# paulmillr/noble-curves

Hardware: AMD Instinct MI355X
Metric: secp256k1_scalar_mults_per_sec (higher is better)
Workload: dtype u32

## Files before the change

### noble-curves_amd/csrc/consts_gen.hpp

```cpp
#pragma once
#include <stdint.h>
namespace ncg {

struct ParamsSecpP {
  static constexpr int N = 8;
  static constexpr uint32_t P[8] = {0xfffffc2fu, 0xfffffffeu, 0xffffffffu, 0xffffffffu, 0xffffffffu, 0xffffffffu, 0xffffffffu, 0xffffffffu};
  static constexpr uint32_t INV = 0xd2253531u;
  static constexpr uint32_t R1[8] = {0x00000001u, 0x00000000u, 0x00000000u, 0x00000000u, 0x00000000u, 0x00000000u, 0x00000000u, 0x00000000u};
  static constexpr uint32_t R2[8] = {0x00000001u, 0x00000000u, 0x00000000u, 0x00000000u, 0x00000000u, 0x00000000u, 0x00000000u, 0x00000000u};
  static constexpr bool TOP_SPARE = false;
  static constexpr bool FOLD = true;
  static constexpr uint32_t FOLD_LO = 0x000003d1u;
  static constexpr uint32_t FOLD_HI = 1u;
  static constexpr int FINAL_SUBS = 1;
  static constexpr uint32_t BETA[8] = {0x719501eeu, 0xc1396c28u, 0x12f58995u, 0x9cf04975u, 0xac3434e9u, 0x6e64479eu, 0x657c0710u, 0x7ae96a2bu};
  static constexpr uint32_t B3[8] = {0x00000015u, 0x00000000u, 0x00000000u, 0x00000000u, 0x00000000u, 0x00000000u, 0x00000000u, 0x00000000u};
};

struct ParamsEdP {
  static constexpr int N = 8;
  static constexpr uint32_t P[8] = {0xffffffedu, 0xffffffffu, 0xffffffffu, 0xffffffffu, 0xffffffffu, 0xffffffffu, 0xffffffffu, 0x7fffffffu};
  static constexpr uint32_t INV = 0x286bca1bu;
  static constexpr uint32_t R1[8] = {0x00000001u, 0x00000000u, 0x00000000u, 0x00000000u, 0x00000000u, 0x00000000u, 0x00000000u, 0x00000000u};
  static constexpr uint32_t R2[8] = {0x00000001u, 0x00000000u, 0x00000000u, 0x00000000u, 0x00000000u, 0x00000000u, 0x00000000u, 0x00000000u};
  static constexpr bool TOP_SPARE = true;
  static constexpr bool FOLD = true;
  static constexpr uint32_t FOLD_LO = 0x00000026u;
  static constexpr uint32_t FOLD_HI = 0u;
  static constexpr int FINAL_SUBS = 2;
  static constexpr uint32_t D[8] = {0x135978a3u, 0x75eb4dcau, 0x4141d8abu, 0x00700a4du, 0x7779e898u, 0x8cc74079u, 0x2b6ffe73u, 0x52036ceeu};
  static constexpr uint32_t D2[8] = {0x26b2f159u, 0xebd69b94u, 0x8283b156u, 0x00e0149au, 0xeef3d130u, 0x198e80f2u, 0x56dffce7u, 0x2406d9dcu};
  static constexpr uint32_t SQRT_M1[8] = {0x4a0ea0b0u, 0xc4ee1b27u, 0xad2fe478u, 0x2f431806u, 0x3dfbd7a7u, 0x2b4d0099u, 0x4fc1df0bu, 0x2b832480u};
};

struct ParamsBlsP {
  static constexpr int N = 12;
  static constexpr uint32_t P[12] = {0xffffaaabu, 0xb9feffffu, 0xb153ffffu, 0x1eabfffeu, 0xf6b0f624u, 0x6730d2a0u, 0xf38512bfu, 0x64774b84u, 0x434bacd7u, 0x4b1ba7b6u, 0x397fe69au, 0x1a0111eau};
  static constexpr uint32_t INV = 0xfffcfffdu;
  static constexpr uint32_t R1[12] = {0x0002fffdu, 0x76090000u, 0xc40c0002u, 0xebf4000bu, 0x53c758bau, 0x5f489857u, 0x70525745u, 0x77ce5853u, 0xa256ec6du, 0x5c071a97u, 0xfa80e493u, 0x15f65ec3u};
  static constexpr uint32_t R2[12] = {0x1c341746u, 0xf4df1f34u, 0x09d104f1u, 0x0a76e6a6u, 0x4c95b6d5u, 0x8de5476cu, 0x939d83c0u, 0x67eb88a9u, 0xb519952du, 0x9a793e85u, 0x92cae3aau, 0x11988fe5u};
  static constexpr bool TOP_SPARE = true;
  static constexpr bool FOLD = false;
};

struct Fe9SecpPR {
  static constexpr uint32_t P[9] = {0x1ffffc2fu, 0x1ffffff7u, 0x1fffffffu, 0x1fffffffu, 0x1fffffffu, 0x1fffffffu, 0x1fffffffu, 0x1fffffffu, 0x00ffffffu};
  static constexpr uint32_t C0 = 31264u, C1 = 256u;
  static constexpr uint32_t PINV = 0x0ddacacfu;
  static constexpr int JMAX = 33;
  static constexpr uint32_t BIAS[8][9] = {
    {0x00000000u, 0x00000000u, 0x00000000u, 0x00000000u, 0x00000000u, 0x00000000u, 0x00000000u, 0x00000000u, 0x00000000u},
    {0x3fff820fu, 0x3ffffef6u, 0x3ffffffeu, 0x3ffffffeu, 0x3ffffffeu, 0x3ffffffeu, 0x3ffffffeu, 0x3ffffffeu, 0x20fffffeu},
    {0x5fff07efu, 0x5ffffdf5u, 0x5ffffffdu, 0x5ffffffdu, 0x5ffffffdu, 0x5ffffffdu, 0x5ffffffdu, 0x5ffffffdu, 0x40fffffdu},
    {0x7ffe8dcfu, 0x7ffffcf4u, 0x7ffffffcu, 0x7ffffffcu, 0x7ffffffcu, 0x7ffffffcu, 0x7ffffffcu, 0x7ffffffcu, 0x60fffffcu},
    {0x9ffe13afu, 0x9ffffbf3u, 0x9ffffffbu, 0x9ffffffbu, 0x9ffffffbu, 0x9ffffffbu, 0x9ffffffbu, 0x9ffffffbu, 0x80fffffbu},
    {0xbffd998fu, 0xbffffaf2u, 0xbffffffau, 0xbffffffau, 0xbffffffau, 0xbffffffau, 0xbffffffau, 0xbffffffau, 0xa0fffffau},
    {0xdffd1f6fu, 0xdffff9f1u, 0xdffffff9u, 0xdffffff9u, 0xdffffff9u, 0xdffffff9u, 0xdffffff9u, 0xdffffff9u, 0xc0fffff9u},
    {0xfffca54fu, 0xfffff8f0u, 0xfffffff8u, 0xfffffff8u, 0xfffffff8u, 0xfffffff8u, 0xfffffff8u, 0xfffffff8u, 0xe0fffff8u},
  };
  static constexpr uint32_t BETA[9] = {0x119501eeu, 0x09cb6143u, 0x1d626570u, 0x0092ea25u, 0x034e99cfu, 0x03cf561au, 0x1c41b991u, 0x056caf80u, 0x007ae96au};
};

struct Fe9EdPR {
  static constexpr uint32_t P[9] = {0x1fffffedu, 0x1fffffffu, 0x1fffffffu, 0x1fffffffu, 0x1fffffffu, 0x1fffffffu, 0x1fffffffu, 0x1fffffffu, 0x007fffffu};
  static constexpr uint32_t C0 = 1216u, C1 = 0u;
  static constexpr uint32_t PINV = 0x179435e5u;
  static constexpr int JMAX = 65;
  static constexpr uint32_t BIAS[8][9] = {
    {0x00000000u, 0x00000000u, 0x00000000u, 0x00000000u, 0x00000000u, 0x00000000u, 0x00000000u, 0x00000000u, 0x00000000u},
    {0x3ffffb2du, 0x3ffffffeu, 0x3ffffffeu, 0x3ffffffeu, 0x3ffffffeu, 0x3ffffffeu, 0x3ffffffeu, 0x3ffffffeu, 0x207ffffeu},
    {0x5ffff66du, 0x5ffffffdu, 0x5ffffffdu, 0x5ffffffdu, 0x5ffffffdu, 0x5ffffffdu, 0x5ffffffdu, 0x5ffffffdu, 0x407ffffdu},
    {0x7ffff1adu, 0x7ffffffcu, 0x7ffffffcu, 0x7ffffffcu, 0x7ffffffcu, 0x7ffffffcu, 0x7ffffffcu, 0x7ffffffcu, 0x607ffffcu},
    {0x9fffecedu, 0x9ffffffbu, 0x9ffffffbu, 0x9ffffffbu, 0x9ffffffbu, 0x9ffffffbu, 0x9ffffffbu, 0x9ffffffbu, 0x807ffffbu},
    {0xbfffe82du, 0xbffffffau, 0xbffffffau, 0xbffffffau, 0xbffffffau, 0xbffffffau, 0xbffffffau, 0xbffffffau, 0xa07ffffau},
    {0xdfffe36du, 0xdffffff9u, 0xdffffff9u, 0xdffffff9u, 0xdffffff9u, 0xdffffff9u, 0xdffffff9u, 0xdffffff9u, 0xc07ffff9u},
    {0xffffdeadu, 0xfffffff8u, 0xfffffff8u, 0xfffffff8u, 0xfffffff8u, 0xfffffff8u, 0xfffffff8u, 0xfffffff8u, 0xe07ffff8u},
  };
  static constexpr uint32_t D[9] = {0x135978a3u, 0x0f5a6e50u, 0x10762addu, 0x00149a82u, 0x1e898007u, 0x003cbbbcu, 0x19ce331du, 0x1dc56dffu, 0x0052036cu};
  static constexpr uint32_t D2[9] = {0x06b2f159u, 0x1eb4dca1u, 0x00ec55bau, 0x00293505u, 0x1d13000eu, 0x00797779u, 0x139c663au, 0x1b8adbffu, 0x002406d9u};
  static constexpr uint32_t SQRT_M1[9] = {0x0a0ea0b0u, 0x0770d93au, 0x0bf91e31u, 0x06300d5au, 0x1d7a72f4u, 0x004c9efdu, 0x1c2cad34u, 0x1009f83bu, 0x002b8324u};
  static constexpr uint32_t SQRT_AD_MINUS_ONE[9] = {0x097b2e1bu, 0x14bfb502u, 0x1e152f5fu, 0x1b1c1836u, 0x1d1fdaf9u, 0x1e6498fau, 0x02b03cf3u, 0x17e57069u, 0x00376931u};
  static constexpr uint32_t INVSQRT_A_MINUS_D[9] = {0x005d40eau, 0x0e47ed54u, 0x105cafa6u, 0x1e2c2eb4u, 0x1d8409d2u, 0x1dc8ff00u, 0x12885b09u, 0x00b9f5ffu, 0x00786c89u};
  static constexpr uint32_t ONE_MINUS_D_SQ[9] = {0x145fc176u, 0x13e04e0cu, 0x178d43f8u, 0x0342719au, 0x0dfe42c8u, 0x15eedf38u, 0x035e6652u, 0x1516567cu, 0x00029072u};
  static constexpr uint32_t D_MINUS_ONE_SQ[9] = {0x04ed4d20u, 0x0d6ad552u, 0x0786664cu, 0x1c945960u, 0x14eebd29u, 0x0997a94du, 0x09053373u, 0x0f5ecd84u, 0x005968b3u};
};

struct ParamsBls29 {
  static constexpr int N = 14;
  static constexpr int BITS = 29;
  static constexpr uint32_t P[14] = {0x1fffaaabu, 0x0ff7ffffu, 0x14ffffeeu, 0x17fffd62u, 0x0f6241eau, 0x09507b58u, 0x0afd9cc3u, 0x109e70a2u, 0x1764774bu, 0x121a5d66u, 0x12c6e9edu, 0x12ffcd34u, 0x00111ea3u, 0x0000000du};
  static constexpr uint32_t INV = 0x1ffcfffdu;
  static constexpr uint32_t R1[14] = {0x03a9fb84u, 0x0ba00690u, 0x071288f1u, 0x0f59bcc5u, 0x126cb614u, 0x0585bf36u, 0x1b85ac3du, 0x1cf856fau, 0x1891ecbdu, 0x1a7eec05u, 0x155a88f0u, 0x0741ac6du, 0x1317c30fu, 0x00000009u};
  static constexpr uint32_t R2[14] = {0x15bef7aeu, 0x1031cd0eu, 0x02dd93e8u, 0x09226323u, 0x0e6e2cd2u, 0x11684daau, 0x1170e5dbu, 0x088e25b1u, 0x1b366399u, 0x1c536f47u, 0x0d1f9cbcu, 0x0278b67fu, 0x1ea66a2bu, 0x0000000cu};
  static constexpr uint32_t PMUL[13][14] = {
    {0x1fffaaabu, 0x0ff7ffffu, 0x14ffffeeu, 0x17fffd62u, 0x0f6241eau, 0x09507b58u, 0x0afd9cc3u, 0x109e70a2u, 0x1764774bu, 0x121a5d66u, 0x12c6e9edu, 0x12ffcd34u, 0x00111ea3u, 0x0000000du},
    {0x1fff5556u, 0x1fefffffu, 0x09ffffdcu, 0x0ffffac5u, 0x1ec483d5u, 0x12a0f6b0u, 0x15fb3986u, 0x013ce144u, 0x0ec8ee97u, 0x0434bacdu, 0x058dd3dbu, 0x05ff9a69u, 0x00223d47u, 0x0000001au},
    {0x1ffeaaacu, 0x1fdfffffu, 0x13ffffb9u, 0x1ffff58au, 0x1d8907aau, 0x0541ed61u, 0x0bf6730du, 0x0279c289u, 0x1d91dd2eu, 0x0869759au, 0x0b1ba7b6u, 0x0bff34d2u, 0x00447a8eu, 0x00000034u},
    {0x1ffd5558u, 0x1fbfffffu, 0x07ffff73u, 0x1fffeb15u, 0x1b120f55u, 0x0a83dac3u, 0x17ece61au, 0x04f38512u, 0x1b23ba5cu, 0x10d2eb35u, 0x16374f6cu, 0x17fe69a4u, 0x0088f51cu, 0x00000068u},
    {0x1ffaaab0u, 0x1f7fffffu, 0x0ffffee7u, 0x1fffd62au, 0x16241eabu, 0x1507b587u, 0x0fd9cc34u, 0x09e70a25u, 0x164774b8u, 0x01a5d66bu, 0x0c6e9ed9u, 0x0ffcd349u, 0x0111ea39u, 0x000000d0u},
    {0x1ff55560u, 0x1effffffu, 0x1ffffdcfu, 0x1fffac54u, 0x0c483d57u, 0x0a0f6b0fu, 0x1fb39869u, 0x13ce144au, 0x0c8ee970u, 0x034bacd7u, 0x18dd3db2u, 0x1ff9a692u, 0x0223d472u, 0x000001a0u},
    {0x1feaaac0u, 0x1dffffffu, 0x1ffffb9fu, 0x1fff58a9u, 0x18907aafu, 0x141ed61eu, 0x1f6730d2u, 0x079c2895u, 0x191dd2e1u, 0x069759aeu, 0x11ba7b64u, 0x1ff34d25u, 0x0447a8e5u, 0x00000340u},
    {0x1fd55580u, 0x1bffffffu, 0x1ffff73fu, 0x1ffeb153u, 0x1120f55fu, 0x083dac3du, 0x1ece61a5u, 0x0f38512bu, 0x123ba5c2u, 0x0d2eb35du, 0x0374f6c8u, 0x1fe69a4bu, 0x088f51cbu, 0x00000680u},
    {0x1faaab00u, 0x17ffffffu, 0x1fffee7fu, 0x1ffd62a7u, 0x0241eabfu, 0x107b587bu, 0x1d9cc34au, 0x1e70a257u, 0x04774b84u, 0x1a5d66bbu, 0x06e9ed90u, 0x1fcd3496u, 0x111ea397u, 0x00000d00u},
    {0x1f555600u, 0x0fffffffu, 0x1fffdcffu, 0x1ffac54fu, 0x0483d57fu, 0x00f6b0f6u, 0x1b398695u, 0x1ce144afu, 0x08ee9709u, 0x14bacd76u, 0x0dd3db21u, 0x1f9a692cu, 0x023d472fu, 0x00001a01u},
    {0x1eaaac00u, 0x1fffffffu, 0x1fffb9feu, 0x1ff58a9fu, 0x0907aaffu, 0x01ed61ecu, 0x16730d2au, 0x19c2895fu, 0x11dd2e13u, 0x09759aecu, 0x1ba7b643u, 0x1f34d258u, 0x047a8e5fu, 0x00003402u},
    {0x1d555800u, 0x1fffffffu, 0x1fff73fdu, 0x1feb153fu, 0x120f55ffu, 0x03dac3d8u, 0x0ce61a54u, 0x138512bfu, 0x03ba5c27u, 0x12eb35d9u, 0x174f6c86u, 0x1e69a4b1u, 0x08f51cbfu, 0x00006804u},
    {0x1aaab000u, 0x1fffffffu, 0x1ffee7fbu, 0x1fd62a7fu, 0x041eabffu, 0x07b587b1u, 0x19cc34a8u, 0x070a257eu, 0x0774b84fu, 0x05d66bb2u, 0x0e9ed90du, 0x1cd34963u, 0x11ea397fu, 0x0000d008u},
  };
  static constexpr uint32_t FOUR[14] = {0x0ea898bau, 0x0e901a40u, 0x124a23e8u, 0x0d66f84fu, 0x0aee547cu, 0x03760629u, 0x181b776eu, 0x12a47aa6u, 0x137ec460u, 0x05c6f549u, 0x0fdc4fe8u, 0x1707174du, 0x0c3ccef5u, 0x0000000cu};
  static constexpr uint32_t G1_BETA[14] = {0x0abf79e7u, 0x194b14ebu, 0x1ceb16a6u, 0x1845cd5du, 0x0c814568u, 0x199ca109u, 0x13ee6ee1u, 0x05d123e5u, 0x0dfbdce2u, 0x010ecb54u, 0x0d9337edu, 0x1daaf4b0u, 0x146806fbu, 0x0000000cu};
  static constexpr uint32_t HALF[14] = {0x01d4fdc2u, 0x15d00348u, 0x13894478u, 0x07acde62u, 0x09365b0au, 0x12c2df9bu, 0x0dc2d61eu, 0x1e7c2b7du, 0x1c48f65eu, 0x0d3f7602u, 0x1aad4478u, 0x13a0d636u, 0x198be187u, 0x00000004u};
  static constexpr uint32_t PSI_X_C0[14] = {0x00000000u, 0x00000000u, 0x00000000u, 0x00000000u, 0x00000000u, 0x00000000u, 0x00000000u, 0x00000000u, 0x00000000u, 0x00000000u, 0x00000000u, 0x00000000u, 0x00000000u, 0x00000000u};
  static constexpr uint32_t PSI_X_C1[14] = {0x154030c4u, 0x16aceb14u, 0x1814e947u, 0x1fba3004u, 0x02e0fc81u, 0x0fb3da4fu, 0x170f2de1u, 0x0acd4cbcu, 0x09689a69u, 0x110b9212u, 0x0533b200u, 0x1554d884u, 0x0ba917a7u, 0x00000000u};
  static constexpr uint32_t PSI_Y_C0[14] = {0x099d9feeu, 0x1cfab983u, 0x07e0b07eu, 0x1f87f0f2u, 0x0bc18573u, 0x0cdbe130u, 0x010ddd19u, 0x100cbeafu, 0x09169c21u, 0x0f93673eu, 0x11de55b3u, 0x097ddc84u, 0x11fce827u, 0x0000000cu};
  static constexpr uint32_t PSI_Y_C1[14] = {0x16620abdu, 0x12fd467cu, 0x0d1f4f6fu, 0x18780c70u, 0x03a0bc76u, 0x1c749a28u, 0x09efbfa9u, 0x0091b1f3u, 0x0e4ddb2au, 0x0286f628u, 0x00e8943au, 0x0981f0b0u, 0x0e14367cu, 0x00000000u};
  static constexpr uint64_t P58[7] = {0x01feffffffffaaabull, 0x02ffffac54ffffeeull, 0x012a0f6b0f6241eaull, 0x0213ce144afd9cc3ull, 0x02434bacd764774bull, 0x025ff9a692c6e9edull, 0x00000001a0111ea3ull};
  static constexpr uint64_t INV58 = 0x01f3fffcfffcfffdull;
};

struct BlsH2c {
  static constexpr int ISO1_XNUM_N = 12;
  static constexpr uint32_t ISO1_XNUM[12][14] = {
    {0x19533850u, 0x1fde0061u, 0x1658849cu, 0x0468a403u, 0x03312074u, 0x0755dadbu, 0x0f9d5f6au, 0x0d765d96u, 0x1f3db0ebu, 0x027072a2u, 0x0cd72ecfu, 0x192a1295u, 0x0b9df03du, 0x00000000u},
    {0x08a13a19u, 0x0e61b7a9u, 0x10c7b287u, 0x19352d6cu, 0x19fcef3au, 0x1bd60694u, 0x0b00008bu, 0x14ac9157u, 0x1bfc81b7u, 0x0cf31437u, 0x1f7ef30cu, 0x174125b4u, 0x16bc996bu, 0x00000003u},
    {0x1d34d585u, 0x001816fdu, 0x0697e05du, 0x0bd01a7fu, 0x06319923u, 0x0526b67eu, 0x127cdfdeu, 0x1c4ccaedu, 0x16999bd6u, 0x1dc05cf6u, 0x0c798715u, 0x1b067cadu, 0x0e1b22d3u, 0x00000001u},
    {0x05b95fd0u, 0x1561eeaeu, 0x0708c4e2u, 0x1ca04592u, 0x0a64d8b5u, 0x161de6c8u, 0x0ed13a80u, 0x1c0b9393u, 0x1f81aea0u, 0x1f7805d0u, 0x1f7443d4u, 0x0410f2d9u, 0x12d9db9fu, 0x00000004u},
    {0x19f42c99u, 0x19554edbu, 0x01bb4832u, 0x08df9f46u, 0x1aa4ed11u, 0x0c014ee5u, 0x0503d165u, 0x024ff2c0u, 0x014d2026u, 0x038449cbu, 0x004265aeu, 0x075ca7f4u, 0x0abdbe88u, 0x0000000cu},
    {0x06e086cbu, 0x12e06cf1u, 0x1010c3f7u, 0x097dc760u, 0x009ce362u, 0x1fdead02u, 0x03b2a43cu, 0x13dc159au, 0x12f1e75fu, 0x0c59d18bu, 0x0993cd0du, 0x17aada76u, 0x0f653a62u, 0x0000000au},
    {0x05f32e93u, 0x04de80d5u, 0x0257dd44u, 0x1b3fa578u, 0x08ad968du, 0x18f7fcf4u, 0x135a2c12u, 0x1b3437dfu, 0x1bf48b7fu, 0x027e482cu, 0x10ad5b95u, 0x1f53c6ecu, 0x13593facu, 0x0000000cu},
    {0x100e8415u, 0x00260d8au, 0x0416be13u, 0x002f5de8u, 0x12f06c69u, 0x0614ac97u, 0x078c4e2cu, 0x0f0e1a44u, 0x12527cbfu, 0x1aa0dad8u, 0x1b9d18c9u, 0x03052990u, 0x06c178c5u, 0x00000008u},
    {0x020e35ffu, 0x1509aba1u, 0x011197a7u, 0x07424063u, 0x00fdf22au, 0x1cdffda5u, 0x15e86ee3u, 0x0dc72f5eu, 0x085ed13bu, 0x17a167e6u, 0x1d4f68a3u, 0x12bc0758u, 0x0da1d102u, 0x0000000bu},
    {0x16f92abfu, 0x1d97eb20u, 0x03799de9u, 0x0afdfcdbu, 0x0593e7abu, 0x1c07c98eu, 0x113c6b21u, 0x0c6c4382u, 0x15178c4bu, 0x004d295bu, 0x160c0213u, 0x0b223d3cu, 0x138a06aeu, 0x00000005u},
    {0x0d584f0eu, 0x13abb276u, 0x114fd2fdu, 0x13587172u, 0x1c078395u, 0x19d77f56u, 0x14ed4ae3u, 0x134b5001u, 0x07368705u, 0x08ccfc06u, 0x169d5582u, 0x04364b97u, 0x1e36a0acu, 0x0000000cu},
    {0x1e2dc07eu, 0x14fb1b8eu, 0x1d54c7fdu, 0x1ffe9f96u, 0x1d9e8c8eu, 0x082c550du, 0x10f80cc9u, 0x0fbb5189u, 0x1731633cu, 0x0d2b8d78u, 0x1142fdc6u, 0x0a530186u, 0x09b1edb4u, 0x00000003u}
  };
  static constexpr int ISO1_XDEN_N = 11;
  static constexpr uint32_t ISO1_XDEN[11][14] = {
    {0x16aada94u, 0x121b61fbu, 0x17d25789u, 0x00ea9a1bu, 0x01f559e5u, 0x1977be06u, 0x17199839u, 0x0b55fcacu, 0x001b9b0eu, 0x101b75ebu, 0x0b9bd0a9u, 0x1276bf47u, 0x14703656u, 0x00000002u},
    {0x109ff044u, 0x10ea0db9u, 0x1f93b8bdu, 0x1ef8d6d2u, 0x1ad8ab3cu, 0x1cd635f7u, 0x1ebd2c90u, 0x01e90c38u, 0x12519856u, 0x1002aed7u, 0x0d3b5c6fu, 0x0cb89003u, 0x0ed3e5c4u, 0x0000000au},
    {0x0f77e4d1u, 0x08f1403du, 0x1b1578a2u, 0x134e8b79u, 0x11c5fe2au, 0x1af37000u, 0x061d1654u, 0x0f79cc45u, 0x1fcafbd1u, 0x00394301u, 0x1c85638fu, 0x02143baau, 0x0fd37998u, 0x00000007u},
    {0x16688f1eu, 0x1834f256u, 0x033c4e2eu, 0x1b7c3ab5u, 0x0aef9a87u, 0x16e2b034u, 0x04ea8170u, 0x0b5ed828u, 0x109f419cu, 0x1b1ce49fu, 0x0b8d1767u, 0x1f6a5c83u, 0x08c7b891u, 0x0000000cu},
    {0x0cfbd1b4u, 0x13f5968cu, 0x04d98113u, 0x078bb5a2u, 0x0a047c3au, 0x1f58a89au, 0x14970a3fu, 0x070dc778u, 0x05a639fau, 0x1e4df2a1u, 0x15236253u, 0x006cbe19u, 0x0747e1aau, 0x00000000u},
    {0x1ba56c55u, 0x0da2285eu, 0x1bdde522u, 0x1323e0bfu, 0x14fcd4dfu, 0x160d9669u, 0x126e3cb8u, 0x1ae38ab4u, 0x043ccd6cu, 0x1c50479du, 0x03ccf828u, 0x14a8dc86u, 0x0baa345eu, 0x00000005u},
    {0x1763cc52u, 0x1af364d0u, 0x0d599836u, 0x01b13b47u, 0x19625c2cu, 0x0c93c70fu, 0x1981cf56u, 0x16ce23d0u, 0x116786d9u, 0x1b64f75fu, 0x0396c2e5u, 0x17ce2455u, 0x137ac25cu, 0x0000000cu},
    {0x135eaa4eu, 0x11a0ee2cu, 0x1c8ae208u, 0x04908755u, 0x0742ff48u, 0x1aa65057u, 0x1ccabcc6u, 0x0ca2e07cu, 0x0a7fdbf0u, 0x065f3fd1u, 0x09b8d593u, 0x11ab564eu, 0x1b009d39u, 0x0000000au},
    {0x04b0c530u, 0x0ab8267du, 0x03c5d708u, 0x0859392au, 0x05ae9638u, 0x1db0f3d5u, 0x0b1bdfc7u, 0x0c8c0cf0u, 0x192090ddu, 0x0f85b4e6u, 0x09cb08bdu, 0x0e6aeeebu, 0x05feaf09u, 0x00000005u},
    {0x0ee55d76u, 0x0fe759f8u, 0x16bac213u, 0x04ced8e4u, 0x097e4bacu, 0x19215e96u, 0x1d46ea21u, 0x145404aeu, 0x11ade63fu, 0x0c8756c9u, 0x031fc337u, 0x15c18a0eu, 0x1fcb94acu, 0x00000005u},
    {0x03a9fb84u, 0x0ba00690u, 0x071288f1u, 0x0f59bcc5u, 0x126cb614u, 0x0585bf36u, 0x1b85ac3du, 0x1cf856fau, 0x1891ecbdu, 0x1a7eec05u, 0x155a88f0u, 0x0741ac6du, 0x1317c30fu, 0x00000009u}
  };
  static constexpr int ISO1_YNUM_N = 16;
// ... 144 lines not shown
```

### noble-curves_amd/csrc/fe9.hpp

```cpp
#pragma once
#include <type_traits>

#include "fp.hpp"
#include "fe9_asm_gen.hpp"
#include "fe9m.hpp"

namespace ncg {

constexpr uint32_t FE9_MASK = (1u << 29) - 1u;

template <class PR, class = void> struct Fe9IsMont : std::false_type {};
template <class PR> struct Fe9IsMont<PR, std::void_t<decltype(PR::MONT)>> : std::integral_constant<bool, PR::MONT> {};

template <class PR>
struct Fe9Raw {
  uint32_t v[9];
};

NCG_DI void fe9_mac(uint64_t& acc, uint32_t a, uint32_t b) {
#ifdef __HIP_DEVICE_COMPILE__
  asm("v_mad_u64_u32 %0, vcc, %1, %2, %0" : "+v"(acc) : "v"(a), "v"(b) : "vcc");
#else
  acc += (uint64_t)a * b;
#endif
// ... 458 lines not shown
  int32_t bw = 0;
#pragma unroll
  for (int i = 0; i < 9; i++) {
    int32_t dd = (int32_t)t[i] - (int32_t)PR::P[i] + bw;
    s[i] = (uint32_t)dd & FE9_MASK;
    bw = dd >> 29;
  }
  const bool ge = bw == 0;
#pragma unroll
  for (int i = 0; i < 9; i++) o[i] = ge ? s[i] : t[i];
}

template <class PR, class... T>
__host__ __device__ __noinline__ bool fe9_eqz_slow(T... limbs) {
  Fe9<PR, 7> a;
  const uint32_t v[9] = {limbs...};
#pragma unroll
  for (int i = 0; i < 9; i++) a.v[i] = v[i];
  uint32_t c[9];
  fe9_canon_limbs<PR, 7>(c, a);
  uint32_t o = 0;
#pragma unroll
  for (int i = 0; i < 9; i++) o |= c[i];
  return o == 0;
}
template <class PR, int A>
NCG_DI bool f_eqz(const Fe9<PR, A>& a) {
  const uint32_t j = (a.v[0] * PR::PINV) & FE9_MASK;
  if (j >= (uint32_t)(PR::JMAX * A)) return false;
  return fe9_eqz_slow<PR>(a.v[0], a.v[1], a.v[2], a.v[3], a.v[4], a.v[5], a.v[6], a.v[7], a.v[8]);
}
template <class PR, int A, int B>
NCG_DI bool f_eq(const Fe9<PR, A>& a, const Fe9<PR, B>& b) {
  return f_eqz(a - b);
}

template <class PR>
NCG_DI Fe9<PR, 1> fe9_from_wire(const uint32_t* __restrict__ p) {
  if constexpr (Fe9IsMont<PR>::value) {
    Fe9<PR, 1> r;
    fe9m_from_wire(r.v, p);
    return r;
  }
  uint32_t w[10];
#pragma unroll
  for (int i = 0; i < 8; i++) w[i] = p[i];
  w[8] = 0;
  w[9] = 0;
  Fe9<PR, 1> r;
#pragma unroll
  for (int i = 0; i < 9; i++) {
    const int bit = 29 * i, limb = bit >> 5, sh = bit & 31;
    const uint64_t two = ((uint64_t)w[limb + 1] << 32) | w[limb];
    r.v[i] = (uint32_t)(two >> sh) & FE9_MASK;
  }
  return r;
}
template <class PR, int A>
NCG_DI void fe9_to_wire(uint32_t* __restrict__ p, const Fe9<PR, A>& a) {
  if constexpr (Fe9IsMont<PR>::value) {
    uint32_t c[9];
    fe9m_canon_plain(c, fe9_norm(a).v);
    fe9m_words_from_limbs(p, c);
    return;
  }
  uint32_t l[11];
  uint32_t c[9];
  fe9_canon_limbs<PR, A>(c, a);
#pragma unroll
  for (int i = 0; i < 9; i++) l[i] = c[i];
  l[9] = 0;
  l[10] = 0;
#pragma unroll
  for (int k = 0; k < 8; k++) {
    const int bit = 32 * k, limb = bit / 29, sh = bit % 29;
    uint64_t acc = (uint64_t)l[limb] >> sh;
    acc |= (uint64_t)l[limb + 1] << (29 - sh);
    acc |= (uint64_t)l[limb + 2] << (58 - sh);
    p[k] = (uint32_t)acc;
  }
}

template <class PR, int A>
NCG_DI Fe9<PR, 1> f_inv(const Fe9<PR, A>& a_in) {
  using F = Fe9<PR, 1>;
  const F x = fe9_norm(a_in);
  if constexpr (Fe9IsMont<PR>::value) {
    F tab[16];
    tab[0] = F::one();
    tab[1] = x;
#pragma unroll
    for (int i = 2; i < 16; i++) tab[i] = tab[i - 1] * x;
    F t = tab[PR::PM2_NIB[63]];
#pragma unroll
    for (int i = 62; i >= 0; i--) {
      t = fe9_sqr_n(t, 4);
      const int d = PR::PM2_NIB[i];
      if (d) t = t * tab[d];
    }
    return t;
  } else if constexpr (PR::C1 != 0) {
    F x2 = f_sqr(x) * x;
    F x3 = f_sqr(x2) * x;
    F x6 = fe9_sqr_n(x3, 3) * x3;
    F x9 = fe9_sqr_n(x6, 3) * x3;
    F x11 = fe9_sqr_n(x9, 2) * x2;
    F x22 = fe9_sqr_n(x11, 11) * x11;
    F x44 = fe9_sqr_n(x22, 22) * x22;
    F x88 = fe9_sqr_n(x44, 44) * x44;
    F x176 = fe9_sqr_n(x88, 88) * x88;
    F x220 = fe9_sqr_n(x176, 44) * x44;
    F x223 = fe9_sqr_n(x220, 3) * x3;
    F t = fe9_sqr_n(x223, 23) * x22;
    t = fe9_sqr_n(t, 5) * x;
    t = fe9_sqr_n(t, 3) * x2;
    t = fe9_sqr_n(t, 2) * x;
    return t;
  } else {
    F z2 = f_sqr(x);
    F z9 = fe9_sqr_n(z2, 2) * x;
    F z11 = z9 * z2;
    F z2_5_0 = f_sqr(z11) * z9;
    F z2_10_0 = fe9_sqr_n(z2_5_0, 5) * z2_5_0;
    F z2_20_0 = fe9_sqr_n(z2_10_0, 10) * z2_10_0;
    F z2_40_0 = fe9_sqr_n(z2_20_0, 20) * z2_20_0;
    F z2_50_0 = fe9_sqr_n(z2_40_0, 10) * z2_10_0;
    F z2_100_0 = fe9_sqr_n(z2_50_0, 50) * z2_50_0;
    F z2_200_0 = fe9_sqr_n(z2_100_0, 100) * z2_100_0;
    F z2_250_0 = fe9_sqr_n(z2_200_0, 50) * z2_50_0;
    return fe9_sqr_n(z2_250_0, 5) * z11;
  }
}

using FeSecp = Fe9<Fe9SecpPR, 2>;
using FeEd = Fe9<Fe9EdPR, 2>;
using FeBn254 = Fe9<Bn254PR, 2>;

}
```

### noble-curves_amd/csrc/hosttest.hip

```cpp
#include <vector>

#include "../../include/ncg.h"
#include "mulvar.hpp"
#include "ed25519.hip"
#include "decode.hip"
#include "ntt.hip"
#include "poly.hip"
#include "h2c.hip"
#include "endo.hpp"
#include "ecdsa.hip"
#include "msm_shard.hpp"
#include "msm_endo.hip"
#include "msm_schedule.hpp"
#include "fe9m_check.hpp"
#include "group_check.hpp"
#include "x25519.hip"
#include "ristretto.hip"

using namespace ncg;

template <class C, int W>
static void ht_mul_var_t(const uint32_t* pts, const uint32_t* scalars, uint32_t* out, uint8_t* out_inf, int n) {
  constexpr int FW = MulVarCfg<C, W>::FW, WW = MulVarCfg<C, W>::WW;
  std::vector<uint32_t> tab(MulVarCfg<C, W>::TS * 2 * FW);
// ... 185 lines not shown
  Fe9<PR, C> z;
  Fe9<PR, D> w;
  for (int i = 0; i < 9; i++) {
    x.v[i] = a[i];
    y.v[i] = b[i];
    z.v[i] = c[i];
    w.v[i] = d[i];
  }
  Fe9<PR, 1> o;
  if constexpr (A * B + C * D <= 7) {
    if (op == 0) o = f_mul_mul(x, y, z, w);
  }
  if constexpr (C <= 2 && A * B + C * C <= 7) {
    if (op == 1) o = f_mul_sqr(x, y, z);
  }
  if constexpr (A * B <= 7) {
    if (op == 2) o = f_mul_add(x, y, z);
  }
  if constexpr (A <= 2) {
    if (op == 3) o = f_sqr_add(x, z);
  }
  if constexpr (A == 1) {
    if (op == 4) {
      const Fe9<PR, 2> h = f_half(x);
      for (int i = 0; i < 9; i++) r[i] = h.v[i];
      return;
    }
  }
  for (int i = 0; i < 9; i++) r[i] = o.v[i];
}
template <class PR>
static int ht_fe9_fused_t(int op, int variant, const uint32_t* a, const uint32_t* b, const uint32_t* c, const uint32_t* d, uint32_t* r) {
  switch (variant) {
    case 1111: ht_fe9_fused_ab<PR, 1, 1, 1, 1>(op, a, b, c, d, r); return 0;
    case 1322: ht_fe9_fused_ab<PR, 1, 3, 2, 2>(op, a, b, c, d, r); return 0;
    case 3211: ht_fe9_fused_ab<PR, 3, 2, 1, 1>(op, a, b, c, d, r); return 0;
    case 2311: ht_fe9_fused_ab<PR, 2, 3, 1, 1>(op, a, b, c, d, r); return 0;
    case 1123: ht_fe9_fused_ab<PR, 1, 1, 2, 3>(op, a, b, c, d, r); return 0;
    case 3121: ht_fe9_fused_ab<PR, 3, 1, 2, 1>(op, a, b, c, d, r); return 0;
    case 1327: ht_fe9_fused_ab<PR, 1, 3, 2, 7>(op, a, b, c, d, r); return 0;
    case 7171: ht_fe9_fused_ab<PR, 7, 1, 7, 1>(op, a, b, c, d, r); return 0;
    case 1771: ht_fe9_fused_ab<PR, 1, 7, 7, 1>(op, a, b, c, d, r); return 0;
    case 2171: ht_fe9_fused_ab<PR, 2, 1, 7, 1>(op, a, b, c, d, r); return 0;
    default: return -1;
  }
}

template <class F>
static int fr29_op_host(int op, const uint32_t* a, const uint32_t* b, uint32_t* r) {
  Fr29 x, y, z;
  for (int i = 0; i < 9; i++) {
    x.v[i] = a[i];
    y.v[i] = b ? b[i] : 0;
    z.v[i] = 0;
  }
  fr29_overflows() = 0;
  switch (op) {
    case 0: z = fr29_mont<F>(x, y); break;
    case 1: z = fr29_add(x, y); break;
    case 2: z = fr29_sub<F>(x, y); break;
    case 3: z = fr29_weak(x); break;
    case 4: z = fr29_reduce256<F>(x); break;
    case 5: z = fr29_cond_sub<F>(x); break;
    case 8: z = fr29_fold255<F>(x); break;
    case 6: {
      uint32_t w[8];
      for (int i = 0; i < 8; i++) w[i] = a[i];
      z = fr29_from_words(w);
      break;
    }
    case 7: {
      uint32_t w[8];
      fr29_to_words(w, x);
      for (int i = 0; i < 8; i++) z.v[i] = w[i];
      z.v[8] = 0;
      break;
    }
    default: return -1;
  }
  for (int i = 0; i < 9; i++) r[i] = z.v[i];
  return fr29_overflows();
}

extern "C" {

int ht_fe9_op(int field, int op, int variant, const uint32_t* a, const uint32_t* b, uint32_t* r) {
  if (field == 0) return ht_fe9_t<Fe9SecpPR>(op, variant, a, b, r);
  if (field == 1) return ht_fe9_t<Fe9EdPR>(op, variant, a, b, r);
  return -1;
}

int ht_mul_var(int curve, const uint32_t* pts, const uint32_t* scalars, uint32_t* out, uint8_t* out_inf, int n) {
  switch (curve) {
    case CURVE_SECP256K1: ht_mul_var_t<CurveSecp, 4>(pts, scalars, out, out_inf, n); return 0;
    case CURVE_BLS12_381_G1: ht_mul_var_t<CurveG1, 3>(pts, scalars, out, out_inf, n); return 0;
    case 12: ht_mul_var_t<CurveG1E, 4>(pts, scalars, out, out_inf, n); return 0;
    case 14: ht_mul_var_t<CurveSecpI, 4>(pts, scalars, out, out_inf, n); return 0;
    case CURVE_BLS12_381_G2: ht_mul_var_t<CurveG2, 3>(pts, scalars, out, out_inf, n); return 0;
    case CURVE_BN254_G1: ht_mul_var_t<CurveBn254, 4>(pts, scalars, out, out_inf, n); return 0;
  }
  return -1;
}

int ht_field_op(int field, int op, const uint32_t* a, const uint32_t* b, uint32_t* r) {
  switch (field) {
    case 0: ht_field_t<ParamsSecpP>(op, a, b, r); return 0;
    case 1: ht_field_t<ParamsEdP>(op, a, b, r); return 0;
    case 2: ht_field_t<ParamsBlsP>(op, a, b, r); return 0;
  }
  return -1;
}

int ht_fe9_fused(int field, int op, int variant, const uint32_t* a, const uint32_t* b, const uint32_t* c, const uint32_t* d,
                 uint32_t* r) {
  if (field == 0) return ht_fe9_fused_t<Fe9SecpPR>(op, variant, a, b, c, d, r);
  if (field == 1) return ht_fe9_fused_t<Fe9EdPR>(op, variant, a, b, c, d, r);
  return -1;
}

int ht_jac_neg(int op, const uint32_t* p, const uint32_t* qx, const uint32_t* qy, uint32_t* out) {
  Jac<FeSecp> P;
  Fe9<Fe9SecpPR, 2> x;
  Fe9<Fe9SecpPR, 3> y;
  for (int i = 0; i < 9; i++) {
    P.X.v[i] = p[i];
    P.Y.v[i] = p[9 + i];
    P.Z.v[i] = p[18 + i];
    x.v[i] = qx[i];
    y.v[i] = qy[i];
  }
  Jac<FeSecp> R;
  if (op == 0) R = jac_dbl_neg(P);
  else if (op == 1) R = jac_madd_neg(P, x, y);
  else return -1;
  for (int i = 0; i < 9; i++) {
    out[i] = R.X.v[i];
    out[9 + i] = R.Y.v[i];
    out[18 + i] = R.Z.v[i];
  }
  return 0;
}

int ht_glv_split_odd(const uint32_t* k, uint32_t* out) {
  uint32_t kk[8];
  for (int i = 0; i < 8; i++) kk[i] = k[i];
  GlvSplit s = secp_glv_split(kk);
  secp_glv_make_odd(s);
  for (int i = 0; i < 5; i++) {
    out[i] = s.k1[i];
    out[5 + i] = s.k2[i];
  }
  out[10] = s.k1neg;
  out[11] = s.k2neg;
  return 0;
}

int ht_glv_split_k1_odd(const uint32_t* k, uint32_t* out) {
  uint32_t kk[8];
  for (int i = 0; i < 8; i++) kk[i] = k[i];
  GlvSplit s = secp_glv_split(kk);
  secp_glv_make_k1_odd(s);
  for (int i = 0; i < 5; i++) {
    out[i] = s.k1[i];
    out[5 + i] = s.k2[i];
  }
  out[10] = s.k1neg;
  out[11] = s.k2neg;
  return 0;
}

int ht_glv_split(const uint32_t* k, uint32_t* out) {
  uint32_t kk[8];
// ... 374 lines not shown
```

Measured before the change: 134.7 million.

## Replace Fermat field inversion with batched divsteps (safegcd) inversion for fe9 fields

Field inversion for non-Montgomery fe9 fields (secp256k1, ed25519) now uses a Bernstein-Yang divsteps algorithm on signed 30-bit limbs. It batches 30 divsteps per iteration with 2x2 transition matrices and exits early once the whole wavefront has g==0, falling back to Fermat inversion if the iteration cap is reached. The aim is to avoid the roughly 256 squarings plus multiplies of exponentiation. The cost is wave-uniform iteration counts and more branchy code. Host test hooks for comparing the two inversions are also added.

After: 136.8 million (median of 6 runs). +1.6%, better.

```diff
diff --git a/noble-curves_amd/csrc/consts_gen.hpp b/noble-curves_amd/csrc/consts_gen.hpp
--- a/noble-curves_amd/csrc/consts_gen.hpp
+++ b/noble-curves_amd/csrc/consts_gen.hpp
@@ -48,6 +48,8 @@
   static constexpr uint32_t C0 = 31264u, C1 = 256u;
   static constexpr uint32_t PINV = 0x0ddacacfu;
   static constexpr int JMAX = 33;
+  static constexpr int32_t P30[9] = {-977, -4, 0, 0, 0, 0, 0, 0, 65536};
+  static constexpr uint32_t PINV30 = 0x2ddacacfu;
   static constexpr uint32_t BIAS[8][9] = {
     {0x00000000u, 0x00000000u, 0x00000000u, 0x00000000u, 0x00000000u, 0x00000000u, 0x00000000u, 0x00000000u, 0x00000000u},
     {0x3fff820fu, 0x3ffffef6u, 0x3ffffffeu, 0x3ffffffeu, 0x3ffffffeu, 0x3ffffffeu, 0x3ffffffeu, 0x3ffffffeu, 0x20fffffeu},
@@ -66,6 +68,8 @@
   static constexpr uint32_t C0 = 1216u, C1 = 0u;
   static constexpr uint32_t PINV = 0x179435e5u;
   static constexpr int JMAX = 65;
+  static constexpr int32_t P30[9] = {-19, 0, 0, 0, 0, 0, 0, 0, 32768};
+  static constexpr uint32_t PINV30 = 0x179435e5u;
   static constexpr uint32_t BIAS[8][9] = {
     {0x00000000u, 0x00000000u, 0x00000000u, 0x00000000u, 0x00000000u, 0x00000000u, 0x00000000u, 0x00000000u, 0x00000000u},
     {0x3ffffb2du, 0x3ffffffeu, 0x3ffffffeu, 0x3ffffffeu, 0x3ffffffeu, 0x3ffffffeu, 0x3ffffffeu, 0x3ffffffeu, 0x207ffffeu},
diff --git a/noble-curves_amd/csrc/fe9.hpp b/noble-curves_amd/csrc/fe9.hpp
--- a/noble-curves_amd/csrc/fe9.hpp
+++ b/noble-curves_amd/csrc/fe9.hpp
@@ -564,7 +564,7 @@
 }
 
 template <class PR, int A>
-NCG_DI Fe9<PR, 1> f_inv(const Fe9<PR, A>& a_in) {
+NCG_DI Fe9<PR, 1> f_inv_fermat(const Fe9<PR, A>& a_in) {
   using F = Fe9<PR, 1>;
   const F x = fe9_norm(a_in);
   if constexpr (Fe9IsMont<PR>::value) {
@@ -614,6 +614,16 @@
   }
 }
 
+}
+#include "fe9_inv.hpp"
+namespace ncg {
+
+template <class PR, int A>
+NCG_DI Fe9<PR, 1> f_inv(const Fe9<PR, A>& a_in) {
+  if constexpr (Fe9IsMont<PR>::value) return f_inv_fermat(a_in);
+  else return fe9_inv_divsteps(a_in);
+}
+
 using FeSecp = Fe9<Fe9SecpPR, 2>;
 using FeEd = Fe9<Fe9EdPR, 2>;
 using FeBn254 = Fe9<Bn254PR, 2>;
diff --git a/noble-curves_amd/csrc/fe9_inv.hpp b/noble-curves_amd/csrc/fe9_inv.hpp
--- /dev/null
+++ b/noble-curves_amd/csrc/fe9_inv.hpp
@@ -0,0 +1,192 @@
+#pragma once
+
+namespace ncg {
+
+constexpr uint32_t FE9_M30 = (1u << 30) - 1u;
+constexpr int FE9_DS_CAP = 20;
+
+NCG_DI bool fe9_wave_any(bool c) {
+#ifdef __HIP_DEVICE_COMPILE__
+  return __builtin_amdgcn_ballot_w64(c) != 0;
+#else
+  return c;
+#endif
+}
+NCG_DI void fe9_ds_fence() {
+#ifdef __HIP_DEVICE_COMPILE__
+  __builtin_amdgcn_sched_barrier(0);
+#endif
+}
+NCG_DI int32_t fe9_mul24(int32_t a, int32_t b) {
+#ifdef __HIP_DEVICE_COMPILE__
+  return __mul24(a, b);
+#else
+  return a * b;
+#endif
+}
+
+struct Fe9DsMat {
+  int32_t u, v, q, r;
+};
+
+NCG_DI Fe9DsMat fe9_divsteps10(int32_t& zeta, uint32_t& f, uint32_t& g) {
+  uint32_t uv = 1u, qr = 1u << 16;
+#pragma unroll
+  for (int i = 0; i < 10; i++) {
+    const uint32_t c1 = (uint32_t)(zeta >> 31);
+    const uint32_t c2 = 0u - (g & 1u);
+    const uint32_t x = (f ^ c1) - c1, y = (uv ^ c1) - c1;
+    g += x & c2;
+    qr += y & c2;
+    const uint32_t c3 = c1 & c2;
+    zeta = (int32_t)(((uint32_t)zeta ^ c3) - 1u);
+    f += g & c3;
+    uv += qr & c3;
+    g >>= 1;
+    uv <<= 1;
+  }
+  Fe9DsMat m;
+  m.u = (int32_t)(int16_t)(uint16_t)uv;
+  m.v = (int32_t)(uv - (uint32_t)m.u) >> 16;
+  m.q = (int32_t)(int16_t)(uint16_t)qr;
+  m.r = (int32_t)(qr - (uint32_t)m.q) >> 16;
+  return m;
+}
+NCG_DI Fe9DsMat fe9_ds_matmul(const Fe9DsMat& b, const Fe9DsMat& a) {
+  Fe9DsMat m;
+  m.u = fe9_mul24(b.u, a.u) + fe9_mul24(b.v, a.q);
+  m.v = fe9_mul24(b.u, a.v) + fe9_mul24(b.v, a.r);
+  m.q = fe9_mul24(b.q, a.u) + fe9_mul24(b.r, a.q);
+  m.r = fe9_mul24(b.q, a.v) + fe9_mul24(b.r, a.r);
+  return m;
+}
+
+NCG_DI void fe9_smac4(int64_t& c0, int64_t& c1, const Fe9DsMat& t, int32_t x, int32_t y) {
+#ifdef __HIP_DEVICE_COMPILE__
+  asm("v_mad_i64_i32 %0, vcc, %2, %6, %0\n\t"
+      "v_mad_i64_i32 %1, vcc, %4, %6, %1\n\t"
+      "v_mad_i64_i32 %0, vcc, %3, %7, %0\n\t"
+      "v_mad_i64_i32 %1, vcc, %5, %7, %1"
+      : "+v"(c0), "+v"(c1)
+      : "v"(t.u), "v"(t.v), "v"(t.q), "v"(t.r), "v"(x), "v"(y)
+      : "vcc");
+#else
+  c0 += (int64_t)t.u * x + (int64_t)t.v * y;
+  c1 += (int64_t)t.q * x + (int64_t)t.r * y;
+#endif
+}
+
+NCG_DI void fe9_ds_update_fg(int32_t (&f)[9], int32_t (&g)[9], const Fe9DsMat& t) {
+  int64_t cf = 0, cg = 0;
+  fe9_smac4(cf, cg, t, f[0], g[0]);
+  cf >>= 30;
+  cg >>= 30;
+#pragma unroll
+  for (int i = 1; i < 9; i++) {
+    fe9_smac4(cf, cg, t, f[i], g[i]);
+    f[i - 1] = (int32_t)((uint32_t)cf & FE9_M30);
+    g[i - 1] = (int32_t)((uint32_t)cg & FE9_M30);
+    cf >>= 30;
+    cg >>= 30;
+  }
+  f[8] = (int32_t)cf;
+  g[8] = (int32_t)cg;
+}
+template <class PR>
+NCG_DI void fe9_ds_update_de(int32_t (&d)[9], int32_t (&e)[9], const Fe9DsMat& t) {
+  const int32_t sd = d[8] >> 31, se = e[8] >> 31;
+  int32_t md = (t.u & sd) + (t.v & se), me = (t.q & sd) + (t.r & se);
+  int64_t cd = 0, ce = 0;
+  fe9_smac4(cd, ce, t, d[0], e[0]);
+  md -= (int32_t)((PR::PINV30 * (uint32_t)cd + (uint32_t)md) & FE9_M30);
+  me -= (int32_t)((PR::PINV30 * (uint32_t)ce + (uint32_t)me) & FE9_M30);
+  cd += (int64_t)PR::P30[0] * md;
+  ce += (int64_t)PR::P30[0] * me;
+  cd >>= 30;
+  ce >>= 30;
+#pragma unroll
+  for (int i = 1; i < 9; i++) {
+    fe9_smac4(cd, ce, t, d[i], e[i]);
+    if (PR::P30[i] != 0) {
+      cd += (int64_t)PR::P30[i] * md;
+      ce += (int64_t)PR::P30[i] * me;
+    }
+    d[i - 1] = (int32_t)((uint32_t)cd & FE9_M30);
+    e[i - 1] = (int32_t)((uint32_t)ce & FE9_M30);
+    cd >>= 30;
+    ce >>= 30;
+  }
+  d[8] = (int32_t)cd;
+  e[8] = (int32_t)ce;
+}
+
+template <class PR>
+NCG_DI void fe9_ds_batch(int32_t& zeta, int32_t (&f)[9], int32_t (&g)[9], int32_t (&d)[9], int32_t (&e)[9]) {
+  uint32_t f0 = (uint32_t)f[0], g0 = (uint32_t)g[0];
+  const Fe9DsMat m1 = fe9_divsteps10(zeta, f0, g0);
+  const Fe9DsMat m2 = fe9_divsteps10(zeta, f0, g0);
+  const Fe9DsMat m3 = fe9_divsteps10(zeta, f0, g0);
+  const Fe9DsMat t = fe9_ds_matmul(m3, fe9_ds_matmul(m2, m1));
+  fe9_ds_fence();
+  fe9_ds_update_de<PR>(d, e, t);
+  fe9_ds_fence();
+  fe9_ds_update_fg(f, g, t);
+  fe9_ds_fence();
+}
+
+template <class PR, int A>
+NCG_DI Fe9<PR, 1> fe9_inv_divsteps(const Fe9<PR, A>& a_in) {
+  uint32_t c[10];
+  {
+    uint32_t cc[9];
+    fe9_canon_limbs<PR, A>(cc, a_in);
+#pragma unroll
+    for (int i = 0; i < 9; i++) c[i] = cc[i];
+    c[9] = 0;
+  }
+  int32_t f[9], g[9], d[9], e[9];
+#pragma unroll
+  for (int i = 0; i < 9; i++) {
+    const int bit = 30 * i, limb = bit / 29, sh = bit % 29;
+    const uint64_t two = ((uint64_t)c[limb + 1] << 29) | c[limb];
+    g[i] = (int32_t)((uint32_t)(two >> sh) & FE9_M30);
+    f[i] = PR::P30[i];
+    d[i] = 0;
+    e[i] = 0;
+  }
+  e[0] = 1;
+  int32_t zeta = -1;
+  uint32_t gnz = 1;
+#pragma unroll 1
+  for (int it = 0; it < FE9_DS_CAP; it++) {
+    fe9_ds_batch<PR>(zeta, f, g, d, e);
+    gnz = 0;
+#pragma unroll
+    for (int i = 0; i < 9; i++) gnz |= (uint32_t)g[i];
+    if (!fe9_wave_any(gnz != 0)) break;
+  }
+  if (gnz != 0) return f_inv_fermat(a_in);
+  const int32_t s = f[8] >> 31;
+  uint32_t w[10];
+  int32_t cy = 0;
+#pragma unroll
+  for (int i = 0; i < 9; i++) {
+    const int32_t t = ((d[i] ^ s) - s) + 2 * PR::P30[i] + cy;
+    w[i] = (uint32_t)t & FE9_M30;
+    cy = t >> 30;
+    if (i == 8) w[i] = (uint32_t)t;
+  }
+  w[9] = 0;
+  Fe9<PR, 1> r;
+#pragma unroll
+  for (int i = 0; i < 9; i++) {
+    const int bit = 29 * i, limb = bit / 30, sh = bit % 30;
+    const uint64_t two = ((uint64_t)w[limb + 1] << 30) | w[limb];
+    r.v[i] = (uint32_t)(two >> sh) & FE9_MASK;
+  }
+  uint32_t o[9];
+  fe9_canon_limbs<PR, 1>(o, r);
+  return Fe9<PR, 1>::from_limbs(o);
+}
+
+}
diff --git a/noble-curves_amd/csrc/hosttest.hip b/noble-curves_amd/csrc/hosttest.hip
--- a/noble-curves_amd/csrc/hosttest.hip
+++ b/noble-curves_amd/csrc/hosttest.hip
@@ -291,12 +291,33 @@
   return fr29_overflows();
 }
 
+template <class PR, int A>
+static void ht_fe9_inv_batch_t(int which, const uint32_t* a, uint32_t* out, uint32_t* raw, int n) {
+  for (int k = 0; k < n; k++) {
+    Fe9<PR, A> x;
+    for (int i = 0; i < 9; i++) x.v[i] = a[(size_t)k * 9 + i];
+    const Fe9<PR, 1> z = which ? f_inv_fermat(x) : f_inv(x);
+    fe9_to_wire(out + (size_t)k * 8, z);
+    if (raw)
+      for (int i = 0; i < 9; i++) raw[(size_t)k * 9 + i] = z.v[i];
+  }
+}
+
 extern "C" {
 
 int ht_fe9_op(int field, int op, int variant, const uint32_t* a, const uint32_t* b, uint32_t* r) {
   if (field == 0) return ht_fe9_t<Fe9SecpPR>(op, variant, a, b, r);
   if (field == 1) return ht_fe9_t<Fe9EdPR>(op, variant, a, b, r);
   return -1;
+}
+
+int ht_fe9_inv_batch(int field, int A, int which, const uint32_t* a, uint32_t* out, uint32_t* raw, int n) {
+  if (field < 0 || field > 1 || (A != 1 && A != 2 && A != 7)) return -1;
+#define CALL(PR) (A == 1 ? ht_fe9_inv_batch_t<PR, 1>(which, a, out, raw, n) : A == 2 ? ht_fe9_inv_batch_t<PR, 2>(which, a, out, raw, n) : ht_fe9_inv_batch_t<PR, 7>(which, a, out, raw, n))
+  if (field == 0) CALL(Fe9SecpPR);
+  else CALL(Fe9EdPR);
+#undef CALL
+  return 0;
 }
 
 int ht_mul_var(int curve, const uint32_t* pts, const uint32_t* scalars, uint32_t* out, uint8_t* out_inf, int n) {
```
